# antoineleeman/robust-nonlinear-mpc

Measured on AMD Instinct MI355X. Metric: QP solves/sec (whole node), rockETH N=20 batch=4096 closed-loop RTI MPC step from script x0, higher is better.
Workload: dtype f64

## Files before the change

__graft_entry__.py:

```python
import os
import subprocess
import sys

ROOT = os.path.dirname(os.path.abspath(__file__))
CSRC = os.path.join(ROOT, "robust-nonlinear-mpc_amd", "csrc")
if ROOT not in sys.path:
    sys.path.insert(0, ROOT)


MFMA_FLAGS = ["-mllvm", "-amdgpu-mfma-vgpr-form"]


def _stale(target, sources):
    if not os.path.exists(target):
        return True
    t = os.path.getmtime(target)
    return any(os.path.getmtime(s) > t for s in sources)


def build(force=False):
    so = os.path.join(CSRC, "libslsqp_hip.so")
    srcs = [os.path.join(CSRC, f) for f in os.listdir(CSRC) if f.endswith((".hip", ".hpp"))] + [os.path.join(ROOT, "include", "slsqp.h")]
    if force or _stale(so, srcs):
        cmd = ["hipcc", "-O3", "--offload-arch=gfx950", "-std=c++17", "-shared", "-fPIC", "-Wno-unused-result", "-Wno-unused-value", "-Wno-pass-failed", *MFMA_FLAGS,
               "-o", so, os.path.join(CSRC, "slsqp_api.hip")] + os.environ.get("SLSQP_EXTRA_FLAGS", "").split()
        subprocess.check_call(cmd)
    so2 = os.path.join(CSRC, "libslsqp_hip_dims62.so")
    if force or _stale(so2, srcs):
        subprocess.check_call(["hipcc", "-O3", "--offload-arch=gfx950", "-std=c++17", "-shared", "-fPIC", "-Wno-unused-result", "-Wno-unused-value", "-Wno-pass-failed", *MFMA_FLAGS,
                               "-DSLSQP_EXTRA_DIMS=X(6,2)", "-o", so2, os.path.join(CSRC, "slsqp_api.hip")])
    from oracle import oracle as O
    O.build(force)
    import robust_nonlinear_mpc_amd
    from robust_nonlinear_mpc_amd import _lib
    import ctypes
    lib = ctypes.CDLL(_lib.SO_PATH)
    missing = [e for e in _lib.EXPORTS if not hasattr(lib, e)]
    if missing:
        raise RuntimeError(f"libslsqp_hip.so lacks symbols: {missing}")


def smoke():
    import numpy as np
    sys.path.insert(0, os.path.join(ROOT, "tests"))
    from problems import make_instance, run_oracle_fastsls, run_gpu_fastsls
    insts = [make_instance("pendulum", s, 0.5) for s in range(4)]
    ref = [run_oracle_fastsls(i, rti_steps=1) for i in insts]
    out = run_gpu_fastsls(insts, rti_steps=1)
    for b, r in enumerate(ref):
        assert bool(out["success"][b]) == bool(r["success"])
        if not r["success"]:
            continue
        err = np.max(np.abs(out["primal_vec"][b] - r["primal_vec"])) / max(1.0, np.max(np.abs(r["primal_vec"])))
        assert err < 1e-6, f"instance {b}: primal mismatch {err}"
        assert np.allclose(out["backoff"][b], r["backoff"], rtol=1e-6, atol=1e-9)
    assert out["success"].any()
    print("smoke ok: max KKT stationarity", float(out["kkt"][:, 0].max()))


if __name__ == "__main__":
    build()
    print("build ok")
```

robust-nonlinear-mpc_amd/csrc/slsqp_kernels.hpp:

```cpp
#pragma once
#include <hip/hip_runtime.h>

#include "dynamics.hpp"
#include "wave_la.hpp"

namespace slsqp {

constexpr double BIGB = 1e19;
__device__ __forceinline__ double nan_max(double a, double b) { return fmax(a, b == b ? b : INFINITY); }
constexpr double EPS_PIN = 1e-10;
constexpr int ST_INIT = -1;

#ifndef NE_MFMA
#define NE_MFMA 1
#endif
#ifndef NE_GJ_MFMA
#define NE_GJ_MFMA 1
#endif

struct Costs {
    const double *Qd, *Rd, *Qfd;
    const double *Qregd, *Rregd, *Qregfd;
    double prox;
};

template <int NX, int NU>
struct Lay {
    static constexpr int NZ = NX + NU, NI = 2 * NZ, NIF = 2 * NX, SR = NX + NI;
    __host__ __device__ static int n(int N) { return NZ * N + NX; }
    __host__ __device__ static int mb(int N) { return N * SR + NIF; }
};

struct QpArgs {
    int B, N;
    const double *A, *Bm;
    const double *q;
    const double *ubg, *lbg;
    const double *x0val;
    const int *run;
    Costs cst;
    double *Linv;
    double *ws;
    double *state;
    double *primal;
    double *dual;
    double *cost;
    double *pin_dual;
    double *kkt;
    int *status, *iters;
    int max_iter;
    double eps;
    double init_s, init_lam;
    int warm_rounds;
    int warm;
    const double *prox;
    int prox_stride;
    unsigned long long *inst_launches;
    int *qpstat;
    int stat_slot;
    int snap_take;
    int snap_use;
    double snap_mu;
    double call_id;
    const double *call_ids;
    int as_first;
    int as_rounds;
    int *diag;
    const int *shift_stepno;
    int warm_shift;
    int as_warm_max_set;
    int as_warm_last;
    double pinf_eps;
    int as_max_viol;
    int n_refine;
    double early_ctol;
};

__host__ __device__ inline size_t kkt_doubles(size_t B) { return 8 * B + 2 + 2 * B; }
__host__ __device__ inline double *x0_record(double *kkt, int B) { return kkt + (size_t)8 * B; }

template <int NX, int NU>
struct QpLds {
    static constexpr int NZ = NX + NU, MM = NX * NX;
    static constexpr bool MFMA = (NE_MFMA != 0) && NX >= 13;
    static constexpr int oA = 0, oL1 = MM, oP = MFMA ? MM : 2 * MM, oQ = oP + MM, oB = oQ + MM, oPiS = oB + NX * NU, oVS = oPiS + NZ + NX,
                         oWp = oVS + NZ + NX, oT1 = oWp + NX, oT2 = oT1 + NX, oT3 = oT2 + NX, TOTAL = oT3 + NX + 1;
};
template <int NX, int NU>
__host__ __device__ constexpr int qp_lds_doubles(int) { return QpLds<NX, NU>::TOTAL; }

__host__ __device__ inline size_t qp_ws_doubles(int n, int N, int NX) { return (size_t)20 * n + (size_t)5 * N * NX; }

template <int NX, int NU>
struct NeG {
    const double *A, *Bm, *ub, *lb;
    double *Linv, *PI, *V, *G, *W;
    double *UF;
    int N;
};

// ... 310 lines not shown
        r.lo = -ub[N * SR + NX + i];
    }
    r.fr = e >= NX;
    r.fu = r.fr && r.hi < BIGB;
    r.fl = r.fr && r.lo > -BIGB;
    return r;
}

enum { P_INIT = 0, P_PRED = 1, P_CORR = 2, P_POL0 = 3, P_POL1 = 4, P_POL2 = 5, P_DONE = 6 };
#ifndef STALL_WINDOW
#define STALL_WINDOW 6
#endif
#ifndef STALL_MIN_IT
#define STALL_MIN_IT 24
#endif
#ifndef STALL_FACTOR
#define STALL_FACTOR 0.5
#endif
#ifndef AS_DELTA
#define AS_DELTA 1e-13
#endif
#ifndef RES_ONLY_TOL
#define RES_ONLY_TOL 1e-9
#endif
struct QpState {
    double phase, it, status, mu, smu, qscale, mtot, pol_round, pol_fail, warm, kst, kbox, ksign, pst, pbox, psign, ticks, fticks, tight, pad;
    double snap_call, snap_mu, snap_used, pad2;
    double mode, cold_as, nviol, path;
    unsigned long long seth[4];
    double kmin, fact_call, act1_ok, uf_valid;
    double res_only, tbox, stall_ref, stall_it;
};
static_assert(sizeof(QpState) == 40 * sizeof(double), "QpState size");

#ifndef LAUNDER_B
#define LAUNDER_B(b) asm volatile("" : "+s"(b))
#endif
template <int NX, int NU>
__device__ __forceinline__ NeG<NX, NU> make_neg(const QpArgs &a, int b) {
    using L = Lay<NX, NU>;
    const int N = a.N, n = L::n(N), mb = L::mb(N);
    double *ws = a.ws + (size_t)b * qp_ws_doubles(n, N, NX);
    NeG<NX, NU> g;
    g.A = a.A + (size_t)b * N * NX * NX; g.Bm = a.Bm + (size_t)b * N * NX * NU;
    g.ub = a.ubg + (size_t)b * mb; g.lb = a.lbg + (size_t)b * mb;
    g.Linv = a.Linv + (size_t)b * N * NX * NX; g.PI = ws + 8 * (size_t)n; g.V = ws + 9 * (size_t)n; g.G = ws + 10 * (size_t)n;
    g.W = ws + 12 * (size_t)n; g.UF = ws + 19 * (size_t)n + 4 * (size_t)N * NX; g.N = N;
    return g;
}

struct FwdPlan { bool factor; double eflag, delta; int k0, ks; };
__device__ __forceinline__ FwdPlan fwd_plan(const QpState *st, int phase, int N) {
    FwdPlan p;
    p.factor = (phase == P_INIT || phase == P_PRED || phase == P_POL0);
    p.eflag = (phase == P_INIT || phase >= P_POL0) ? 1.0 : 0.0;
    p.delta = (phase == P_POL0 || (phase == P_INIT && st->mode == 0.0)) ? AS_DELTA : 0.0;
    p.k0 = (phase == P_POL0) ? (int)st->kmin : 0;
    p.ks = (phase == P_POL0 && st->uf_valid != 0.0 && p.k0 < N) ? p.k0 : 0;
    return p;
}

__device__ __noinline__ int x0_gate(double *kkt, int B, int b, int slot, double vmax, int lane) {
    double *xr = x0_record(kkt, B);
    if (lane == 0) xr[2 + (size_t)b * 2 + slot] = vmax;
    return (vmax > fmax(1e-9, xr[0]) || !(vmax < INFINITY)) ? 1 : 0;
}

template <int NX, int NU>
__device__ __forceinline__ void phase_update(const QpArgs &a, int first, int b, int lane, double *sm = nullptr) {
    using L = Lay<NX, NU>;
    constexpr int NZ = L::NZ, SR = L::SR;
    const int N = a.N, n = L::n(N), mb = L::mb(N);
    const double *ub = a.ubg + (size_t)b * mb, *qg = a.q + (size_t)b * n;
    double *ws = a.ws + (size_t)b * qp_ws_doubles(n, N, NX);
    double *Z = ws, *SU = Z + n, *SL = SU + n, *LU = SL + n, *LL = LU + n, *GC = LL + n, *CU = GC + n, *CL = CU + n;
    double *PI = CL + n, *V = PI + n, *G = V + n, *ACT = G + n, *W = ACT + n, *NUA = W + N * NX, *NUP = NUA + N * NX;
    double *SZ = NUP + N * NX, *SSU = SZ + n, *SSL = SSU + n, *SLU = SSL + n, *SLL = SLU + n, *SGC = SLL + n, *SNUA = SGC + n;
    double *ACT1 = SNUA + N * NX;
    double *ACT2 = ws + 19 * (size_t)n + 5 * (size_t)N * NX;
    Costs cst = a.cst;
    cst.prox = a.prox ? a.prox[(size_t)b * a.prox_stride] : 0.0;
    const double call_id = a.call_ids ? a.call_ids[b] : a.call_id;
    QpState *stp = (QpState *)a.state + b;
    auto restore_iterate = [&](double mu_snap) {
        const double smin = fmax(sqrt(fmax(mu_snap, 0.0)), 1e-3);
#pragma unroll 4
        for (int e = lane; e < n; e += 64) {
            const Elem el = elem_of<NX, NU>(e, n, N, ub, qg, cst);
            const double z = (e < NX) ? a.x0val[(size_t)b * NX + e] : SZ[e], su = SSU[e], sl = SSL[e];
            Z[e] = z; GC[e] = SGC[e];
            SU[e] = el.fu ? fmax(el.hi - z, fmin(su, smin)) : 1.0; LU[e] = el.fu ? SLU[e] : 0.0;
            SL[e] = el.fl ? fmax(z - el.lo, fmin(sl, smin)) : 1.0; LL[e] = el.fl ? SLL[e] : 0.0;
        }
        for (int o = lane; o < N * NX; o += 64) NUA[o] = SNUA[o];
    };

    if (first) {
        int status = ST_INIT;
        double viol = -INFINITY;
        if (lane < NX) {
            const double xv = a.x0val[(size_t)b * NX + lane];
            viol = fmax(xv - ub[NX + lane], -ub[NX + NZ + lane] - xv);
            if (isnan(viol)) viol = INFINITY;
        }
        if (x0_gate(a.kkt, a.B, b, a.stat_slot, wla::wave_max(viol), lane)) status = 2;
        int okbits = (int)stp->act1_ok;
        int age1 = (okbits >> 2) & 255, age2 = (okbits >> 10) & 255;
        if (a.stat_slot == 0 && a.snap_use == 0 && a.warm_shift && (!a.shift_stepno || a.shift_stepno[b] > 0)) { age1 = min(age1 + 1, 255); age2 = min(age2 + 1, 255); }
        okbits = (okbits & 3) | (age1 << 2) | (age2 << 10);
        const bool from_act1 = a.warm && status == ST_INIT && a.stat_slot == 0 && a.snap_use == 0 && (okbits & 1);
        bool warm = a.warm && status == ST_INIT && (from_act1 || (((int)stp->status == 0) && ((int)stp->phase == P_DONE)));
        const bool have_act2 = a.warm && status == ST_INIT && a.stat_slot == 1 && a.as_warm_last > 0 && (okbits & 2);
        bool from_act2 = have_act2 && (a.as_warm_last >= 2 || !warm);
        bool big_set = false;
        if (warm && !from_act1 && !from_act2 && a.snap_use != 0 && a.as_warm_max_set > 0) {
            double cnt = 0.0;
            for (int e = lane; e < n; e += 64) cnt += (ACT[e] != 0.0) ? 1.0 : 0.0;
            big_set = wla::wave_sum(cnt) > (double)a.as_warm_max_set;
            if (big_set) { if (have_act2) { from_act2 = true; big_set = false; } else warm = false; }
        }
        if (from_act2) warm = true;
        const double *prev = a.primal + (size_t)b * n;
        const bool keep_fact = warm && !from_act1 && !from_act2 && a.snap_use != 0 && stp->fact_call == call_id && call_id != 0.0;
        double set_changed = 0.0;
        double qscale = 0.0, mtot = 0.0;
#pragma unroll 4
        for (int e = lane; e < n; e += 64) {
            const Elem el = elem_of<NX, NU>(e, n, N, ub, qg, cst);
            qscale = fmax(qscale, fabs(el.q));
            mtot += (el.fu ? 1.0 : 0.0) + (el.fl ? 1.0 : 0.0);
            if (warm) {
                const double ac_old = ACT[e];
                const double *src = from_act1 ? ACT1 : ACT2;
                int es = e + (from_act1 ? age1 : age2) * NZ;
                while (es >= n) es -= NZ;
                double ac = (from_act1 || from_act2) ? src[es] : ac_old;
                if ((ac > 0.0 && !el.fu) || (ac < 0.0 && !el.fl) || !el.fr) ac = 0.0;
                if (ac != ac_old) set_changed = 1.0;
                const double zp = (e < NX) ? a.x0val[(size_t)b * NX + e] : prev[e];
                const double z0 = ac > 0.0 ? el.hi : (ac < 0.0 ? el.lo : zp);
                const double pi = (el.fr && ac == 0.0) ? wla::fast_rcp(el.pd) : 0.0;
                ACT[e] = ac; PI[e] = pi; V[e] = (pi != 0.0) ? -pi * el.q : z0;
            } else {
                const double z0 = (e < NX) ? a.x0val[(size_t)b * NX + e] : 0.0;
                const double pi = el.fr ? wla::fast_rcp(el.pd) : 0.0;
                PI[e] = pi; V[e] = (pi != 0.0) ? -pi * el.q : z0; Z[e] = z0;
            }
        }
        qscale = fmax(1.0, wla::wave_max(qscale));
        mtot = fmax(1.0, wla::wave_sum(mtot));
        const bool skip_fact = keep_fact && wla::wave_max(set_changed) == 0.0;
        if (lane == 0) {
            QpState s0;
            s0.phase = (status == ST_INIT) ? (warm ? P_POL0 : P_INIT) : P_DONE; s0.it = 0; s0.status = status; s0.mu = 0; s0.smu = 0; s0.qscale = qscale;
            s0.mtot = mtot; s0.pol_round = 0; s0.pol_fail = 0; s0.warm = warm ? 1.0 : 0.0; s0.kst = 0; s0.kbox = 0; s0.ksign = 0; s0.pst = -1; s0.pbox = -1; s0.psign = -1; s0.ticks = 0; s0.fticks = 0; s0.tight = 0; s0.pad = 0;
            s0.snap_call = stp->snap_call; s0.snap_mu = stp->snap_mu; s0.snap_used = 0; s0.pad2 = 0;
            s0.mode = (a.as_first && !big_set) ? 0.0 : 1.0; s0.cold_as = big_set ? 1.0 : 0.0; s0.nviol = 0; s0.path = warm ? (from_act2 ? 20.0 : 10.0) : (big_set ? 1.0 : 0.0);
            s0.seth[0] = s0.seth[1] = s0.seth[2] = s0.seth[3] = 0ULL; s0.kmin = skip_fact ? (double)N : 0.0; s0.fact_call = 0; s0.act1_ok = (double)okbits; s0.uf_valid = 0; s0.res_only = 0; s0.tbox = 0; s0.stall_ref = 0; s0.stall_it = 0;
            *stp = s0;
            a.status[b] = status; a.iters[b] = 0;
#ifdef QP_DIAG_SPAN
            if (a.diag) for (int i = 0; i < 32; i++) a.diag[((size_t)b * 2 + a.stat_slot) * 32 + i] = -1;
#endif
            if (status != ST_INIT && a.qpstat) {
                int *qs = a.qpstat + ((size_t)b * 2 + a.stat_slot) * 8;
                for (int i = 0; i < 8; i++) qs[i] = 0;
                qs[6] = status;
            }
        }
        return;
    }

    QpState s = *stp;
    int phase = (int)s.phase;
    if (phase == P_DONE) return;
    int status = (int)s.status, it = (int)s.it;
    const double qscale = s.qscale, mtot = s.mtot, ptol = 1e-9 * qscale;
    double tol = (s.tight != 0.0 ? fmin(a.eps, 1e-9) : a.eps) * qscale;
    bool polished = false, start_iter = false, fall_back = false;

    bool as_from_init = false;
    if (phase == P_INIT && s.mode == 0.0) {
#pragma unroll 4
        for (int e = lane; e < n; e += 64) {
            const Elem el = elem_of<NX, NU>(e, n, N, ub, qg, cst);
            const double gc = G[e];
            CU[e] = el.fr ? -(el.q + gc) * wla::fast_rcp(el.pd) : Z[e];
            CL[e] = gc; ACT[e] = 0.0;
        }
        for (int o = lane; o < N * NX; o += 64) NUP[o] = W[o];
        s.cold_as = 1.0; s.warm = 2.0; s.pol_round = 0.0; s.pol_fail = 0.0; s.nviol = 0.0;
        as_from_init = true;
        phase = P_POL0;
        wla::wsync_mem();
    }
    if (phase == P_INIT) {
        for (int o = lane; o < N * NX; o += 64) NUA[o] = W[o];
#pragma unroll 4
        for (int e = lane; e < n; e += 64) {
            const Elem el = elem_of<NX, NU>(e, n, N, ub, qg, cst);
            const double gc = G[e];
            const double z = el.fr ? -(el.q + gc) * wla::fast_rcp(el.pd) : Z[e];
            GC[e] = gc; Z[e] = z;
            const double lam0 = a.init_lam > 0.0 ? a.init_lam : fmax(1.0, 0.1 * qscale);
            SU[e] = el.fu ? fmax(el.hi - z, a.init_s) : 1.0; LU[e] = el.fu ? lam0 : 0.0;
            SL[e] = el.fl ? fmax(z - el.lo, a.init_s) : 1.0; LL[e] = el.fl ? lam0 : 0.0;
        }
        start_iter = true;
    } else if (phase == P_PRED) {
        double amin = 1.0, S0 = 0.0, S1 = 0.0, S2 = 0.0;
#pragma unroll 4
        for (int e = lane; e < n; e += 64) {
            const Elem el = elem_of<NX, NU>(e, n, N, ub, qg, cst);
            const double dz = V[e] - PI[e] * G[e];
            const double z = Z[e], su = SU[e], sl = SL[e], lu = LU[e], ll = LL[e];
            double cu = 0.0, cl = 0.0;
            if (el.fu) {
                const double ru = z + su - el.hi, dsu = -ru - dz, dlu = -lu + (lu * ru + lu * dz) * wla::fast_rcp(su);
                if (dsu < 0) amin = fmin(amin, -su * wla::fast_rcp(dsu));
                if (dlu < 0) amin = fmin(amin, -lu * wla::fast_rcp(dlu));
                S0 += su * lu; S1 += su * dlu + lu * dsu; cu = dsu * dlu; S2 += cu;
            }
            if (el.fl) {
                const double rl = el.lo - z + sl, dsl = -rl + dz, dll = -ll + (ll * rl - ll * dz) * wla::fast_rcp(sl);
                if (dsl < 0) amin = fmin(amin, -sl * wla::fast_rcp(dsl));
                if (dll < 0) amin = fmin(amin, -ll * wla::fast_rcp(dll));
                S0 += sl * ll; S1 += sl * dll + ll * dsl; cl = dsl * dll; S2 += cl;
            }
            CU[e] = cu; CL[e] = cl;
        }
        const double aaff = wla::wave_min(amin);
        S0 = wla::wave_sum(S0); S1 = wla::wave_sum(S1); S2 = wla::wave_sum(S2);
        const double muaff = (S0 + aaff * (S1 + aaff * S2)) / mtot;
        double sig = muaff / s.mu; sig = sig * sig * sig;
        const double smu = sig * s.mu;
        s.smu = smu;
#pragma unroll 4
        for (int e = lane; e < n; e += 64) {
            const Elem el = elem_of<NX, NU>(e, n, N, ub, qg, cst);
            const double z = Z[e], su = SU[e], sl = SL[e], lu = LU[e], ll = LL[e];
            double rr = el.fr ? el.pd * z + el.q + GC[e] + lu - ll : 0.0;
            if (el.fu) rr += (-(su * lu + CU[e] - smu) + lu * (z + su - el.hi)) * wla::fast_rcp(su);
            if (el.fl) rr -= (-(sl * ll + CL[e] - smu) + ll * (el.lo - z + sl)) * wla::fast_rcp(sl);
            V[e] = -PI[e] * rr;
        }
        phase = P_CORR;
    } else if (phase == P_CORR) {
        const double smu = s.smu;
        double amin = 1e300;
#pragma unroll 4
        for (int e = lane; e < n; e += 64) {
            const Elem el = elem_of<NX, NU>(e, n, N, ub, qg, cst);
            const double dz = V[e] - PI[e] * G[e];
            const double z = Z[e], su = SU[e], sl = SL[e], lu = LU[e], ll = LL[e];
            if (el.fu) {
                const double ru = z + su - el.hi, dsu = -ru - dz;
                const double dlu = (-(su * lu + CU[e] - smu) + lu * ru + lu * dz) * wla::fast_rcp(su);
                if (dsu < 0) amin = fmin(amin, -su * wla::fast_rcp(dsu));
                if (dlu < 0) amin = fmin(amin, -lu * wla::fast_rcp(dlu));
            }
            if (el.fl) {
                const double rl = el.lo - z + sl, dsl = -rl + dz;
                const double dll = (-(sl * ll + CL[e] - smu) + ll * rl - ll * dz) * wla::fast_rcp(sl);
                if (dsl < 0) amin = fmin(amin, -sl * wla::fast_rcp(dsl));
                if (dll < 0) amin = fmin(amin, -ll * wla::fast_rcp(dll));
            }
        }
        const double alpha = fmin(1.0, 0.99 * wla::wave_min(amin));
#pragma unroll 4
        for (int e = lane; e < n; e += 64) {
            const Elem el = elem_of<NX, NU>(e, n, N, ub, qg, cst);
            const double gg = G[e];
            const double dz = V[e] - PI[e] * gg;
            const double z = Z[e], su = SU[e], sl = SL[e], lu = LU[e], ll = LL[e];
            if (el.fu) {
                const double ru = z + su - el.hi, dsu = -ru - dz;
                const double dlu = (-(su * lu + CU[e] - smu) + lu * ru + lu * dz) * wla::fast_rcp(su);
                SU[e] = su + alpha * dsu; LU[e] = lu + alpha * dlu;
            }
            if (el.fl) {
                const double rl = el.lo - z + sl, dsl = -rl + dz;
                const double dll = (-(sl * ll + CL[e] - smu) + ll * rl - ll * dz) * wla::fast_rcp(sl);
                SL[e] = sl + alpha * dsl; LL[e] = ll + alpha * dll;
            }
            Z[e] = z + alpha * dz; GC[e] += alpha * gg;
        }
        for (int o = lane; o < N * NX; o += 64) NUA[o] += alpha * W[o];
        it++;
        start_iter = true;
    } else if (phase == P_POL2 && s.res_only != 0.0 && stp->pbox < RES_ONLY_TOL * qscale) {
        polished = true; status = 0; s.kst = s.pst; s.kbox = s.tbox; s.ksign = s.psign; s.pbox = stp->pbox; s.res_only = 0.0;
        phase = P_DONE;
    } else {
        s.res_only = 0.0;
        const bool firstp = (phase == P_POL0);
        const double max_rounds = (s.warm == 1.0) ? (double)a.warm_rounds : (s.warm == 2.0 ? (double)a.as_rounds : 8.0);
        const bool look = (phase == P_POL0 && s.pol_fail == 0.0 && s.pol_round < max_rounds);
        const bool fused_look = look && sm != nullptr;
        if (!as_from_init && !fused_look) {
#pragma unroll 4
            for (int e = lane; e < n; e += 64) {
                const double gg = G[e];
                CU[e] = V[e] - PI[e] * gg;
                CL[e] = (firstp ? 0.0 : CL[e]) + gg;
            }
            for (int o = lane; o < N * NX; o += 64) NUP[o] = (firstp ? 0.0 : NUP[o]) + W[o];
            wla::wsync_mem();
        }
        auto viol_at = [&](int e, double tolv) -> double {
            if (e < NX || e >= n || ACT[e] != 0.0) return 0.0;
            const Elem el = elem_of<NX, NU>(e, n, N, ub, qg, cst);
            const double zn = CU[e];
            double v = 0.0;
            if (el.fu) v = fmax(v, zn - el.hi);
            if (el.fl) v = fmax(v, el.lo - zn);
            return v > tolv ? v : 0.0;
        };
        auto plan_set = [&](double tolv, double &nv, unsigned long long &hash) -> double {
            int in_viol = 0;
            for (int o = lane; o < N * NU; o += 64) {
                const int e = (o / NU) * NZ + NX + (o % NU);
                in_viol |= (viol_at(e, tolv) > 0.0) ? 1 : 0;
            }
            const bool any_in = wla::wave_or(in_viol) != 0;
            double changed = 0.0, viols = 0.0, kfirst = 1e9;
            unsigned long long hv = 0ULL;
#pragma unroll 2
            for (int e = lane; e < n; e += 64) {
                const Elem el = elem_of<NX, NU>(e, n, N, ub, qg, cst);
                const double zn = CU[e], gr = el.pd * zn + el.q + CL[e], ac = ACT[e];
                double nac = ac;
                if (ac > 0.0 && gr > tolv) nac = 0.0;
                if (ac < 0.0 && -gr > tolv) nac = 0.0;
                if (ac == 0.0 && el.fr) {
                    const double vu = el.fu ? zn - el.hi : 0.0, vl = el.fl ? el.lo - zn : 0.0, v = fmax(vu, vl);
                    if (v > tolv) {
                        viols += 1.0;
                        bool take = true;
                        if ((e % NZ) < NX) take = !any_in && (v >= viol_at(e - NZ, tolv)) && (v >= viol_at(e + NZ, tolv));
                        if (take) nac = vu > vl ? 1.0 : -1.0;
                    }
                }
                if (nac != ac) { changed += 1.0; kfirst = fmin(kfirst, (double)max(0, e / NZ - ((e % NZ) < NX ? 1 : 0))); }
                if (nac != 0.0) {
                    unsigned long long x = (unsigned long long)(2 * e + (nac > 0.0 ? 1 : 0)) + 0x9E3779B97F4A7C15ULL;
                    x = (x ^ (x >> 30)) * 0xBF58476D1CE4E5B9ULL; x = (x ^ (x >> 27)) * 0x94D049BB133111EBULL; hv ^= x ^ (x >> 31);
                }
                G[e] = nac;
            }
#pragma unroll
            for (int o = 32; o > 0; o >>= 1) {
                const unsigned lo32 = __shfl_xor((unsigned)(hv & 0xFFFFFFFFULL), o), hi32 = __shfl_xor((unsigned)(hv >> 32), o);
                hv ^= ((unsigned long long)hi32 << 32) | lo32;
            }
            hash = hv | 1ULL;
            nv = wla::wave_sum(viols);
            s.kmin = fmin(wla::wave_min(kfirst), (double)N);
            return wla::wave_sum(changed);
        };
        auto seen_before = [&](unsigned long long hsh) -> bool {
            const bool rep = (hsh == s.seth[0]) || (hsh == s.seth[1]) || (hsh == s.seth[2]) || (hsh == s.seth[3]);
            s.seth[3] = s.seth[2]; s.seth[2] = s.seth[1]; s.seth[1] = s.seth[0]; s.seth[0] = hsh;
            return rep;
        };
        auto apply_set = [&]() {
            wla::wsync_mem();
#pragma unroll 4
            for (int e = lane; e < n; e += 64) {
                const Elem el = elem_of<NX, NU>(e, n, N, ub, qg, cst);
                const double zn = CU[e], ac = G[e];
                const double z0 = ac > 0.0 ? el.hi : (ac < 0.0 ? el.lo : zn);
                const double pi = (el.fr && ac == 0.0) ? wla::fast_rcp(el.pd) : 0.0;
                ACT[e] = ac; PI[e] = pi; V[e] = (pi != 0.0) ? -pi * el.q : z0;
            }
        };
        bool again = false, give_up = false;
        double tvst = 0.0, tvbox = 0.0, tvsign = 0.0;
        auto fused_plan = [&](double tolv, double &nv, unsigned long long &hash) -> double {
            double *sV = sm, *sN = sm + n;
            int in_viol = 0;
            double viols = 0.0;
#pragma unroll 2
            for (int e = lane; e < n; e += 64) {
                const Elem el = elem_of<NX, NU>(e, n, N, ub, qg, cst);
                double zn, cl;
                if (as_from_init) { zn = CU[e]; cl = CL[e]; }
                else {
                    const double gg = G[e];
                    zn = V[e] - PI[e] * gg; cl = (firstp ? 0.0 : CL[e]) + gg;
                    CU[e] = zn; CL[e] = cl;
                }
                const double gr = el.pd * zn + el.q + cl, ac = ACT[e];
                if (el.fr && ac == 0.0) tvst = nan_max(tvst, fabs(gr));
                if (el.fu) tvbox = nan_max(tvbox, zn - el.hi);
                if (el.fl) tvbox = nan_max(tvbox, el.lo - zn);
                if (ac > 0.0) tvsign = nan_max(tvsign, gr);
                if (ac < 0.0) tvsign = nan_max(tvsign, -gr);
                double nac = ac;
                if (ac > 0.0 && gr > tolv) nac = 0.5;
                if (ac < 0.0 && -gr > tolv) nac = 0.5;
                double v = 0.0;
                if (ac == 0.0 && el.fr) {
                    const double vu = el.fu ? zn - el.hi : 0.0, vl = el.fl ? el.lo - zn : 0.0, vm = fmax(vu, vl);
                    if (vm > tolv) { v = vu > vl ? vm : -vm; viols += 1.0; if ((e % NZ) >= NX) in_viol = 1; }
                }
                sV[e] = v; sN[e] = nac;
            }
            if (!as_from_init) for (int o = lane; o < N * NX; o += 64) NUP[o] = (firstp ? 0.0 : NUP[o]) + W[o];
            wla::wsync();
            const bool any_in = wla::wave_or(in_viol) != 0;
            double changed = 0.0, kfirst = 1e9;
#ifdef QP_DIAG_SPAN
            double klast = -1.0;
#endif
            unsigned long long hv = 0ULL;
#pragma unroll 2
            for (int e = lane; e < n; e += 64) {
                const double v = sV[e];
                double nac = sN[e];
                bool chg = (nac == 0.5);
                if (chg) nac = 0.0;
                if (v != 0.0) {
                    bool take = true;
                    if ((e % NZ) < NX) {
                        const double va = fabs(v), vp = (e - NZ >= NX) ? fabs(sV[e - NZ]) : 0.0, vn = (e + NZ < n) ? fabs(sV[e + NZ]) : 0.0;
                        take = !any_in && va >= vp && va >= vn;
                    }
                    if (take) { nac = v > 0.0 ? 1.0 : -1.0; chg = true; }
                }
                if (chg) { changed += 1.0; kfirst = fmin(kfirst, (double)max(0, e / NZ - ((e % NZ) < NX ? 1 : 0))); }
#ifdef QP_DIAG_SPAN
                if (chg) klast = fmax(klast, (double)min(N - 1, e / NZ));
#endif
                if (nac != 0.0) {
                    unsigned long long x = (unsigned long long)(2 * e + (nac > 0.0 ? 1 : 0)) + 0x9E3779B97F4A7C15ULL;
                    x = (x ^ (x >> 30)) * 0xBF58476D1CE4E5B9ULL; x = (x ^ (x >> 27)) * 0x94D049BB133111EBULL; hv ^= x ^ (x >> 31);
                }
                sN[e] = nac;
            }
#pragma unroll
            for (int o = 32; o > 0; o >>= 1) {
                const unsigned lo32 = __shfl_xor((unsigned)(hv & 0xFFFFFFFFULL), o), hi32 = __shfl_xor((unsigned)(hv >> 32), o);
                hv ^= ((unsigned long long)hi32 << 32) | lo32;
            }
            hash = hv | 1ULL;
            nv = wla::wave_sum(viols);
            s.kmin = fmin(wla::wave_min(kfirst), (double)N);
#ifdef QP_DIAG_SPAN
            {
                const double kl = wla::wave_max(klast);
                const int r = (int)s.pol_round;
                if (lane == 0 && a.diag && r < 16 && kl >= 0.0) { int *dg = a.diag + (((size_t)b * 2 + a.stat_slot) * 16 + r) * 2; dg[0] = (int)s.kmin; dg[1] = (int)kl; }
            }
#endif
            return wla::wave_sum(changed);
        };
        auto fused_apply = [&]() {
            const double *sN = sm + n;
#pragma unroll 4
            for (int e = lane; e < n; e += 64) {
                const Elem el = elem_of<NX, NU>(e, n, N, ub, qg, cst);
                const double ac = sN[e];
                const double z0 = ac > 0.0 ? el.hi : (ac < 0.0 ? el.lo : 0.0);
                const double pi = (el.fr && ac == 0.0) ? wla::fast_rcp(el.pd) : 0.0;
                ACT[e] = ac; PI[e] = pi; V[e] = (pi != 0.0) ? -pi * el.q : ((e < NX) ? a.x0val[(size_t)b * NX + e] : z0);
            }
        };
        if (look) {
            double nv = 0.0;
            unsigned long long hsh = 0ULL;
            const double changed = fused_look ? fused_plan(a.early_ctol * qscale, nv, hsh) : plan_set(a.early_ctol * qscale, nv, hsh);
            again = changed > 0.0;
            if (again && s.warm > 0.0 && seen_before(hsh)) { again = false; give_up = true; }
            if (s.warm > 0.0 && (nv > (double)a.as_max_viol || (s.pol_round > 0.0 && nv > 2.0 * s.nviol + 8.0 && nv > 24.0))) { again = false; give_up = true; }
            s.nviol = nv;
            if (again) { s.pol_round += 1.0; if (fused_look) fused_apply(); else apply_set(); s.uf_valid = 1.0; }
            if (fused_look) wla::wsync_mem();
        } else if (phase == P_POL0 && s.warm > 0.0) give_up = true;
        if (again) {
            phase = P_POL0;
        } else if (give_up) {
            fall_back = true;
        } else if (phase != P_POL2) {
    #pragma unroll 4
        for (int e = lane; e < n; e += 64) {
                const Elem el = elem_of<NX, NU>(e, n, N, ub, qg, cst);
                const double pi = PI[e], zn = CU[e];
                const double r1 = (pi != 0.0) ? el.pd * zn + el.q + CL[e] : 0.0;
                V[e] = zn - pi * r1;
            }
            s.res_only = 0.0;
            if (fused_look && a.n_refine <= 1 && s.pol_fail == 0.0) {
                const double wst = wla::wave_max(tvst), wbox = wla::wave_max(tvbox), wsign = wla::wave_max(tvsign);
                if (wst < ptol && wbox < ptol && wsign < ptol) { s.res_only = 1.0; s.pst = wst; s.tbox = wbox; s.psign = wsign; }
            }
            if (phase == P_POL0) { s.pad = 0.0; phase = (a.n_refine <= 1) ? P_POL2 : P_POL1; }
            else { s.pad += 1.0; phase = (s.pad + 1.0 >= (double)a.n_refine) ? P_POL2 : P_POL1; }
        } else {
            double vst = 0.0, vbox = 0.0, vsign = 0.0;
    #pragma unroll 4
        for (int e = lane; e < n; e += 64) {
                const Elem el = elem_of<NX, NU>(e, n, N, ub, qg, cst);
                const double zn = CU[e], gr = el.pd * zn + el.q + CL[e], ac = ACT[e];
                if (el.fr && ac == 0.0) vst = nan_max(vst, fabs(gr));
                if (el.fu) vbox = nan_max(vbox, zn - el.hi);
                if (el.fl) vbox = nan_max(vbox, el.lo - zn);
                if (ac > 0.0) vsign = nan_max(vsign, gr);
                if (ac < 0.0) vsign = nan_max(vsign, -gr);
            }
            vst = wla::wave_max(vst); vbox = wla::wave_max(vbox); vsign = wla::wave_max(vsign);
            s.pst = vst; s.psign = vsign;
            const bool pf = s.pol_fail != 0.0;
            const double eqres = stp->pbox;
            s.pbox = eqres;
            if (!pf && vst < ptol && vbox < ptol && vsign < ptol && eqres < 1e-6 * qscale) {
                polished = true; status = 0; s.kst = vst; s.kbox = vbox; s.ksign = vsign;
                phase = P_DONE;
            } else if (!pf && vst < ptol && s.pol_round < max_rounds) {
                double nv = 0.0;
                unsigned long long hsh = 0ULL;
                plan_set(ptol, nv, hsh);
                if (s.warm > 0.0 && seen_before(hsh)) fall_back = true;
                else { s.pol_round += 1.0; s.nviol = nv; apply_set(); phase = P_POL0; s.uf_valid = 0.0; }
            } else if (s.warm > 0.0) {
                fall_back = true;
            } else if (s.tight == 0.0 && a.eps > 1e-9 && status == 4) {
                s.tight = 1.0; s.pol_round = 0.0; s.pol_fail = 0.0; tol = fmin(a.eps, 1e-9) * qscale;
                start_iter = true;
            } else phase = P_DONE;
        }
    }

    if (fall_back) {
        const bool try_cold_as = a.as_first == 1 && s.cold_as == 0.0 && s.warm == 1.0;
        s.pol_round = 0.0; s.pol_fail = 0.0; s.seth[0] = s.seth[1] = s.seth[2] = s.seth[3] = 0ULL; s.uf_valid = 0.0;
        if (!try_cold_as && a.snap_use && s.snap_call == call_id && call_id != 0.0) {
            s.warm = -1.0; s.path = 10.0 * floor(s.path / 10.0) + 2.0;
            restore_iterate(s.snap_mu);
            s.snap_used = 1.0;
            start_iter = true;
        } else {
            const double w10 = 10.0 * floor(s.path / 10.0);
            if (try_cold_as) { s.mode = 0.0; s.path = w10 + 3.0; s.warm = -1.0; }
            else { s.mode = 1.0; s.path = w10 + 1.0; s.warm = -1.0; }
    #pragma unroll 4
            for (int e = lane; e < n; e += 64) {
                const Elem el = elem_of<NX, NU>(e, n, N, ub, qg, cst);
                const double z0 = (e < NX) ? a.x0val[(size_t)b * NX + e] : 0.0;
                const double pi = el.fr ? wla::fast_rcp(el.pd) : 0.0;
                PI[e] = pi; V[e] = (pi != 0.0) ? -pi * el.q : z0; Z[e] = z0;
            }
            phase = P_INIT;
        }
    }

    if (start_iter) {
        wla::wsync_mem();
        double rmax = 0.0, musum = 0.0;
#pragma unroll 4
        for (int e = lane; e < n; e += 64) {
            const Elem el = elem_of<NX, NU>(e, n, N, ub, qg, cst);
            const double z = Z[e], su = SU[e], sl = SL[e], lu = LU[e], ll = LL[e];
            const double rd = el.fr ? el.pd * z + el.q + GC[e] + lu - ll : 0.0;
            const double ru = el.fu ? z + su - el.hi : 0.0, rl = el.fl ? el.lo - z + sl : 0.0;
            rmax = fmax(rmax, fmax(fabs(rd), fmax(fabs(ru), fabs(rl))));
            musum += (el.fu ? su * lu : 0.0) + (el.fl ? sl * ll : 0.0);
            const double Wu = el.fu ? lu * wla::fast_rcp(su) : 0.0, Wl = el.fl ? ll * wla::fast_rcp(sl) : 0.0;
            const double pi = el.fr ? wla::fast_rcp(el.pd + Wu + Wl) : 0.0;
            const double tu = el.fu ? -lu + Wu * ru : 0.0, tl = el.fl ? -ll + Wl * rl : 0.0;
            PI[e] = pi; V[e] = -pi * (rd + tu - tl);
        }
        const double res = wla::wave_max(rmax);
        const double mu = wla::wave_sum(musum) / mtot;
        s.mu = mu; s.kst = res;
        bool farkas = false;
        if (a.pinf_eps > 0.0 && it >= 4 && res == res) {
            double ymax = 0.0, aty = 0.0, sup = 0.0;
#pragma unroll 4
            for (int e = lane; e < n; e += 64) {
                const Elem el = elem_of<NX, NU>(e, n, N, ub, qg, cst);
                const double lu = el.fu ? LU[e] : 0.0, ll = el.fl ? LL[e] : 0.0, gc = GC[e];
                ymax = fmax(ymax, fmax(lu, ll));
                if (el.fr) { aty = fmax(aty, fabs(gc + lu - ll)); sup += (el.fu ? el.hi * lu : 0.0) - (el.fl ? el.lo * ll : 0.0); }
                else sup -= a.x0val[(size_t)b * NX + e] * gc;
            }
            const double *lbv = a.lbg + (size_t)b * mb;
            for (int o = lane; o < N * NX; o += 64) {
                const double nu = NUA[o];
                const int r = (o / NX) * SR + (o % NX);
                ymax = fmax(ymax, fabs(nu));
                sup += 0.5 * (ub[r] + lbv[r]) * nu;
            }
            ymax = wla::wave_max(ymax); aty = wla::wave_max(aty); sup = wla::wave_sum(sup);
            farkas = ymax > 0.0 && aty <= a.pinf_eps * ymax && sup < -a.pinf_eps * ymax;
        }
        if (a.snap_take && s.pad2 == 0.0 && mu <= a.snap_mu * qscale && mu >= 1e-2 * a.snap_mu * qscale && res == res) {
#pragma unroll 4
            for (int e = lane; e < n; e += 64) { SZ[e] = Z[e]; SSU[e] = SU[e]; SSL[e] = SL[e]; SLU[e] = LU[e]; SLL[e] = LL[e]; SGC[e] = GC[e]; }
            for (int o = lane; o < N * NX; o += 64) SNUA[o] = NUA[o];
            s.pad2 = 1.0; s.snap_call = call_id; s.snap_mu = mu;
        }
        bool stalled = false;
        {
            const double phi = fmax(res, mu);
            if (s.stall_ref == 0.0) { s.stall_ref = phi; s.stall_it = (double)it; }
            else if ((double)it - s.stall_it >= (double)STALL_WINDOW) {
                stalled = it >= STALL_MIN_IT && phi > STALL_FACTOR * s.stall_ref;
                s.stall_ref = phi; s.stall_it = (double)it;
            }
        }
        if (farkas) { status = 5; phase = P_DONE; }
        else if (!(res == res) || !(mu == mu) || res > 1e30) { status = 3; phase = P_DONE; }
        else if (res < tol && mu < tol) {
            status = 4;
    #pragma unroll 4
        for (int e = lane; e < n; e += 64) {
                const Elem el = elem_of<NX, NU>(e, n, N, ub, qg, cst);
                const double z = Z[e], lam = LU[e] - LL[e];
                const bool aU = el.fu && (lam > el.hi - z);
                const bool aL = el.fl && !aU && (-lam > z - el.lo);
                const double z0 = aU ? el.hi : (aL ? el.lo : z);
                const double pi = (el.fr && !aU && !aL) ? wla::fast_rcp(el.pd) : 0.0;
                ACT[e] = aU ? 1.0 : (aL ? -1.0 : 0.0); PI[e] = pi; V[e] = (pi != 0.0) ? -pi * el.q : z0;
            }
            phase = P_POL0; s.kmin = 0.0; s.uf_valid = 0.0;
        } else if (it >= a.max_iter || stalled) {
            status = (s.tight != 0.0 && status == 4) ? 4 : 1; phase = P_DONE;
        }
        else phase = P_PRED;
    }

    if (phase == P_DONE) {
        wla::wsync_mem();
        double *pr = a.primal + (size_t)b * n, *du = a.dual + (size_t)b * mb;
        double csum = 0.0, nact = 0.0;
        const bool ok = (status == 0 || status == 4);
        if (ok) {
    #pragma unroll 4
        for (int e = lane; e < n; e += 64) {
                const Elem el = elem_of<NX, NU>(e, n, N, ub, qg, cst);
                double zv, yu, yl, gv;
                if (polished) {
                    zv = CU[e]; gv = CL[e];
                    const double gr = el.pd * zv + el.q + gv, ac = ACT[e];
                    yu = ac > 0.0 ? fmax(-gr, 0.0) : 0.0;
                    yl = ac < 0.0 ? fmax(gr, 0.0) : 0.0;
                } else { zv = Z[e]; gv = GC[e]; yu = el.fu ? LU[e] : 0.0; yl = el.fl ? LL[e] : 0.0; }
                pr[e] = zv;
                nact += (yu > 0.0 ? 1.0 : 0.0) + (yl > 0.0 ? 1.0 : 0.0);
                csum += 0.5 * el.pd * zv * zv + el.q * zv;
                const int k = e / NZ, i = e % NZ;
                if (k < N) { du[k * SR + NX + i] = yu; du[k * SR + NX + NZ + i] = yl; }
                else { du[N * SR + i] = yu; du[N * SR + NX + i] = yl; }
                if (e < NX && a.pin_dual) a.pin_dual[(size_t)b * NX + e] = -(el.pd * zv + el.q + gv);
            }
            const double *nus = polished ? NUP : NUA;
            for (int o = lane; o < N * NX; o += 64) du[(o / NX) * SR + (o % NX)] = nus[o];
            if (polished && a.stat_slot == 0 && a.snap_use == 0) {
                for (int e = lane; e < n; e += 64) ACT1[e] = ACT[e];
                s.act1_ok = (double)((((int)s.act1_ok | 1)) & ~(255 << 2));
            }
            if (polished && a.stat_slot == 1) {
                for (int e = lane; e < n; e += 64) ACT2[e] = ACT[e];
                s.act1_ok = (double)((((int)s.act1_ok | 2)) & ~(255 << 10));
            }
        }
        if (polished) s.fact_call = call_id;
        csum = wla::wave_sum(csum);
        nact = wla::wave_sum(nact);
        if (lane == 0) {
            if (a.qpstat) {
                int *qs = a.qpstat + ((size_t)b * 2 + a.stat_slot) * 8;
                qs[0] = it; qs[1] = (int)stp->ticks; qs[2] = (int)stp->fticks; qs[3] = (int)nact; qs[4] = (int)s.path / 10;
                qs[5] = (int)s.pol_round; qs[6] = status; qs[7] = (int)s.path % 10;
            }
            if (ok) a.cost[b] = csum;
            a.status[b] = status;
            a.iters[b] = it;
            double *kk = a.kkt + (size_t)b * 8;
            kk[0] = s.kst; kk[1] = s.kbox; kk[2] = s.ksign; kk[3] = s.mu; kk[4] = s.pst; kk[5] = s.pbox; kk[6] = stp->fticks; kk[7] = stp->ticks;
        }
    }
    if (lane == 0) { s.phase = phase; s.it = it; s.status = status; s.ticks = stp->ticks; s.fticks = stp->fticks; *stp = s; }
}

#ifndef QP_PERSIST_WAVES_PER_SIMD
#define QP_PERSIST_WAVES_PER_SIMD 3
#endif

template <int NX, int NU, bool MX = false>
__device__ __forceinline__ int qp_solve_dev(const QpArgs &a, int b, int lane, double *sm, int max_ticks, int resume = 0, unsigned long long deadline = ~0ULL,
                                            const unsigned *fin_count = nullptr, unsigned cut_count = 0xFFFFFFFFu) {
    if (!resume) {
        if (a.run && !a.run[b]) {
            if (a.qpstat && lane < 8) a.qpstat[((size_t)b * 2 + a.stat_slot) * 8 + lane] = (lane == 6) ? -1 : 0;
            return 1;
        }
// ... 1229 lines not shown
```

Measured before the change: 1.538 million.

## Fuse IPM iterate update with residual and Farkas passes in QP phase update

The interior-point iterate update (init, predictor step, snapshot restore) now computes residuals, complementarity sums, the PI/V factors and the Farkas infeasibility statistics in the same per-element loop, so the separate re-read passes are skipped. The polishing correction also folds the V refinement into the plan loop and reuses the fused plan/apply for refinement rounds. The aim is fewer global memory sweeps over the workspace per IPM iteration. In exchange it adds register pressure, extra wave syncs before snapshot and polish loops, and subtle ordering changes such as the Farkas test now using the post-increment iteration count. An unfused build is kept behind a macro.

```diff
diff --git a/__graft_entry__.py b/__graft_entry__.py
--- a/__graft_entry__.py
+++ b/__graft_entry__.py
@@ -29,6 +29,10 @@
     if force or _stale(so2, srcs):
         subprocess.check_call(["hipcc", "-O3", "--offload-arch=gfx950", "-std=c++17", "-shared", "-fPIC", "-Wno-unused-result", "-Wno-unused-value", "-Wno-pass-failed", *MFMA_FLAGS,
                                "-DSLSQP_EXTRA_DIMS=X(6,2)", "-o", so2, os.path.join(CSRC, "slsqp_api.hip")])
+    so3 = os.path.join(CSRC, "libslsqp_hip_unfused.so")
+    if force or _stale(so3, srcs):
+        subprocess.check_call(["hipcc", "-O3", "--offload-arch=gfx950", "-std=c++17", "-shared", "-fPIC", "-Wno-unused-result", "-Wno-unused-value", "-Wno-pass-failed", *MFMA_FLAGS,
+                               "-DQP_FUSED_PASSES=0", "-o", so3, os.path.join(CSRC, "slsqp_api.hip")])
     from oracle import oracle as O
     O.build(force)
     import robust_nonlinear_mpc_amd
diff --git a/robust-nonlinear-mpc_amd/csrc/slsqp_kernels.hpp b/robust-nonlinear-mpc_amd/csrc/slsqp_kernels.hpp
--- a/robust-nonlinear-mpc_amd/csrc/slsqp_kernels.hpp
+++ b/robust-nonlinear-mpc_amd/csrc/slsqp_kernels.hpp
@@ -16,6 +16,9 @@
 #endif
 #ifndef NE_GJ_MFMA
 #define NE_GJ_MFMA 1
+#endif
+#ifndef QP_FUSED_PASSES
+#define QP_FUSED_PASSES 1
 #endif
 
 struct Costs {
@@ -492,6 +495,7 @@
     cst.prox = a.prox ? a.prox[(size_t)b * a.prox_stride] : 0.0;
     const double call_id = a.call_ids ? a.call_ids[b] : a.call_id;
     QpState *stp = (QpState *)a.state + b;
+#if !QP_FUSED_PASSES
     auto restore_iterate = [&](double mu_snap) {
         const double smin = fmax(sqrt(fmax(mu_snap, 0.0)), 1e-3);
 #pragma unroll 4
@@ -504,6 +508,7 @@
         }
         for (int o = lane; o < N * NX; o += 64) NUA[o] = SNUA[o];
     };
+#endif
 
     if (first) {
         int status = ST_INIT;
@@ -589,6 +594,50 @@
     double tol = (s.tight != 0.0 ? fmin(a.eps, 1e-9) : a.eps) * qscale;
     bool polished = false, start_iter = false, fall_back = false;
 
+#if QP_FUSED_PASSES
+    double it_rmax = 0.0, it_musum = 0.0, fk_ymax = 0.0, fk_aty = 0.0, fk_sup = 0.0;
+    bool iter_ready = false, fk_on = false;
+    auto iter_begin = [&]() __attribute__((always_inline)) { iter_ready = true; fk_on = a.pinf_eps > 0.0 && it >= 4; asm volatile("" : "+v"(lane)); };
+    auto iter_elem = [&](int e, const Elem &el, double z, double su, double sl, double lu, double ll, double gc) __attribute__((always_inline)) {
+        const double rd = el.fr ? el.pd * z + el.q + gc + lu - ll : 0.0;
+        const double ru = el.fu ? z + su - el.hi : 0.0, rl = el.fl ? el.lo - z + sl : 0.0;
+        it_rmax = fmax(it_rmax, fmax(fabs(rd), fmax(fabs(ru), fabs(rl))));
+        it_musum += (el.fu ? su * lu : 0.0) + (el.fl ? sl * ll : 0.0);
+        const double Wu = el.fu ? lu * wla::fast_rcp(su) : 0.0, Wl = el.fl ? ll * wla::fast_rcp(sl) : 0.0;
+        const double pi = el.fr ? wla::fast_rcp(el.pd + Wu + Wl) : 0.0;
+        const double tu = el.fu ? -lu + Wu * ru : 0.0, tl = el.fl ? -ll + Wl * rl : 0.0;
+        PI[e] = pi; V[e] = -pi * (rd + tu - tl);
+        if (fk_on) {
+            const double flu = el.fu ? lu : 0.0, fll = el.fl ? ll : 0.0;
+            fk_ymax = fmax(fk_ymax, fmax(flu, fll));
+            if (el.fr) { fk_aty = fmax(fk_aty, fabs(gc + flu - fll)); fk_sup += (el.fu ? el.hi * flu : 0.0) - (el.fl ? el.lo * fll : 0.0); }
+            else fk_sup -= a.x0val[(size_t)b * NX + e] * gc;
+        }
+    };
+    auto iter_nu = [&](int o, double nu) __attribute__((always_inline)) {
+        if (fk_on) {
+            const double *lbv = a.lbg + (size_t)b * mb;
+            const int r = (o / NX) * SR + (o % NX);
+            fk_ymax = fmax(fk_ymax, fabs(nu));
+            fk_sup += 0.5 * (ub[r] + lbv[r]) * nu;
+        }
+    };
+    auto restore_iterate = [&](double mu_snap) __attribute__((always_inline)) {
+        const double smin = fmax(sqrt(fmax(mu_snap, 0.0)), 1e-3);
+        iter_begin();
+#pragma unroll 1
+        for (int e = lane; e < n; e += 64) {
+            const Elem el = elem_of<NX, NU>(e, n, N, ub, qg, cst);
+            const double z = (e < NX) ? a.x0val[(size_t)b * NX + e] : SZ[e], su = SSU[e], sl = SSL[e], gc = SGC[e];
+            const double sun = el.fu ? fmax(el.hi - z, fmin(su, smin)) : 1.0, lun = el.fu ? SLU[e] : 0.0;
+            const double sln = el.fl ? fmax(z - el.lo, fmin(sl, smin)) : 1.0, lln = el.fl ? SLL[e] : 0.0;
+            Z[e] = z; GC[e] = gc; SU[e] = sun; LU[e] = lun; SL[e] = sln; LL[e] = lln;
+            iter_elem(e, el, z, sun, sln, lun, lln, gc);
+        }
+        for (int o = lane; o < N * NX; o += 64) { const double nu = SNUA[o]; NUA[o] = nu; iter_nu(o, nu); }
+    };
+#endif
+
     bool as_from_init = false;
     if (phase == P_INIT && s.mode == 0.0) {
 #pragma unroll 4
@@ -605,6 +654,21 @@
         wla::wsync_mem();
     }
     if (phase == P_INIT) {
+#if QP_FUSED_PASSES
+        iter_begin();
+        const double lam0 = a.init_lam > 0.0 ? a.init_lam : fmax(1.0, 0.1 * qscale);
+#pragma unroll 1
+        for (int e = lane; e < n; e += 64) {
+            const Elem el = elem_of<NX, NU>(e, n, N, ub, qg, cst);
+            const double gc = G[e];
+            const double z = el.fr ? -(el.q + gc) * wla::fast_rcp(el.pd) : Z[e];
+            const double su = el.fu ? fmax(el.hi - z, a.init_s) : 1.0, lu = el.fu ? lam0 : 0.0;
+            const double sl = el.fl ? fmax(z - el.lo, a.init_s) : 1.0, ll = el.fl ? lam0 : 0.0;
+            GC[e] = gc; Z[e] = z; SU[e] = su; LU[e] = lu; SL[e] = sl; LL[e] = ll;
+            iter_elem(e, el, z, su, sl, lu, ll, gc);
+        }
+        for (int o = lane; o < N * NX; o += 64) { const double nu = W[o]; NUA[o] = nu; iter_nu(o, nu); }
+#else
         for (int o = lane; o < N * NX; o += 64) NUA[o] = W[o];
 #pragma unroll 4
         for (int e = lane; e < n; e += 64) {
@@ -616,6 +680,7 @@
             SU[e] = el.fu ? fmax(el.hi - z, a.init_s) : 1.0; LU[e] = el.fu ? lam0 : 0.0;
             SL[e] = el.fl ? fmax(z - el.lo, a.init_s) : 1.0; LL[e] = el.fl ? lam0 : 0.0;
         }
+#endif
         start_iter = true;
     } else if (phase == P_PRED) {
         double amin = 1.0, S0 = 0.0, S1 = 0.0, S2 = 0.0;
@@ -677,6 +742,34 @@
             }
         }
         const double alpha = fmin(1.0, 0.99 * wla::wave_min(amin));
+#if QP_FUSED_PASSES
+        it++;
+        iter_begin();
+#pragma unroll 2
+        for (int e = lane; e < n; e += 64) {
+            const Elem el = elem_of<NX, NU>(e, n, N, ub, qg, cst);
+            const double gg = G[e];
+            const double dz = V[e] - PI[e] * gg;
+            const double z = Z[e];
+            double su = SU[e], sl = SL[e], lu = LU[e], ll = LL[e];
+            if (el.fu) {
+                const double ru = z + su - el.hi, dsu = -ru - dz;
+                const double dlu = (-(su * lu + CU[e] - smu) + lu * ru + lu * dz) * wla::fast_rcp(su);
+                su = su + alpha * dsu; lu = lu + alpha * dlu;
+                SU[e] = su; LU[e] = lu;
+            }
+            if (el.fl) {
+                const double rl = el.lo - z + sl, dsl = -rl + dz;
+                const double dll = (-(sl * ll + CL[e] - smu) + ll * rl - ll * dz) * wla::fast_rcp(sl);
+                sl = sl + alpha * dsl; ll = ll + alpha * dll;
+                SL[e] = sl; LL[e] = ll;
+            }
+            const double zn = z + alpha * dz, gc = GC[e] + alpha * gg;
+            Z[e] = zn; GC[e] = gc;
+            iter_elem(e, el, zn, su, sl, lu, ll, gc);
+        }
+        for (int o = lane; o < N * NX; o += 64) { const double nu = NUA[o] + alpha * W[o]; NUA[o] = nu; iter_nu(o, nu); }
+#else
 #pragma unroll 4
         for (int e = lane; e < n; e += 64) {
             const Elem el = elem_of<NX, NU>(e, n, N, ub, qg, cst);
@@ -697,6 +790,7 @@
         }
         for (int o = lane; o < N * NX; o += 64) NUA[o] += alpha * W[o];
         it++;
+#endif
         start_iter = true;
     } else if (phase == P_POL2 && s.res_only != 0.0 && stp->pbox < RES_ONLY_TOL * qscale) {
         polished = true; status = 0; s.kst = s.pst; s.kbox = s.tbox; s.ksign = s.psign; s.pbox = stp->pbox; s.res_only = 0.0;
@@ -786,21 +880,36 @@
         };
         bool again = false, give_up = false;
         double tvst = 0.0, tvbox = 0.0, tvsign = 0.0;
-        auto fused_plan = [&](double tolv, double &nv, unsigned long long &hash) -> double {
+        auto fused_plan = [&](double tolv, double &nv, unsigned long long &hash, bool corr = false) -> double {
             double *sV = sm, *sN = sm + n;
             int in_viol = 0;
             double viols = 0.0;
+            const bool have_zn = as_from_init || corr;
 #pragma unroll 2
             for (int e = lane; e < n; e += 64) {
                 const Elem el = elem_of<NX, NU>(e, n, N, ub, qg, cst);
                 double zn, cl;
-                if (as_from_init) { zn = CU[e]; cl = CL[e]; }
+#if QP_FUSED_PASSES
+                double pi;
+                if (have_zn) { zn = CU[e]; cl = CL[e]; pi = PI[e]; }
+                else {
+                    const double gg = G[e];
+                    pi = PI[e];
+                    zn = V[e] - pi * gg; cl = (firstp ? 0.0 : CL[e]) + gg;
+                    CU[e] = zn; CL[e] = cl;
+                }
+#else
+                if (have_zn) { zn = CU[e]; cl = CL[e]; }
                 else {
                     const double gg = G[e];
                     zn = V[e] - PI[e] * gg; cl = (firstp ? 0.0 : CL[e]) + gg;
                     CU[e] = zn; CL[e] = cl;
                 }
+#endif
                 const double gr = el.pd * zn + el.q + cl, ac = ACT[e];
+#if QP_FUSED_PASSES
+                V[e] = zn - pi * ((pi != 0.0) ? gr : 0.0);
+#endif
                 if (el.fr && ac == 0.0) tvst = nan_max(tvst, fabs(gr));
                 if (el.fu) tvbox = nan_max(tvbox, zn - el.hi);
                 if (el.fl) tvbox = nan_max(tvbox, el.lo - zn);
@@ -860,12 +969,12 @@
             {
                 const double kl = wla::wave_max(klast);
                 const int r = (int)s.pol_round;
-                if (lane == 0 && a.diag && r < 16 && kl >= 0.0) { int *dg = a.diag + (((size_t)b * 2 + a.stat_slot) * 16 + r) * 2; dg[0] = (int)s.kmin; dg[1] = (int)kl; }
+                if (lane == 0 && a.diag && r < 16 && kl >= 0.0 && !corr) { int *dg = a.diag + (((size_t)b * 2 + a.stat_slot) * 16 + r) * 2; dg[0] = (int)s.kmin; dg[1] = (int)kl; }
             }
 #endif
             return wla::wave_sum(changed);
         };
-        auto fused_apply = [&]() {
+        auto fused_apply = [&](bool corr = false) {
             const double *sN = sm + n;
 #pragma unroll 4
             for (int e = lane; e < n; e += 64) {
@@ -873,7 +982,7 @@
                 const double ac = sN[e];
                 const double z0 = ac > 0.0 ? el.hi : (ac < 0.0 ? el.lo : 0.0);
                 const double pi = (el.fr && ac == 0.0) ? wla::fast_rcp(el.pd) : 0.0;
-                ACT[e] = ac; PI[e] = pi; V[e] = (pi != 0.0) ? -pi * el.q : ((e < NX) ? a.x0val[(size_t)b * NX + e] : z0);
+                ACT[e] = ac; PI[e] = pi; V[e] = (pi != 0.0) ? -pi * el.q : ((e < NX) ? (corr ? CU[e] : a.x0val[(size_t)b * NX + e]) : z0);
             }
         };
         if (look) {
@@ -892,12 +1001,14 @@
         } else if (give_up) {
             fall_back = true;
         } else if (phase != P_POL2) {
+            if (!(QP_FUSED_PASSES && fused_look)) {
     #pragma unroll 4
         for (int e = lane; e < n; e += 64) {
                 const Elem el = elem_of<NX, NU>(e, n, N, ub, qg, cst);
                 const double pi = PI[e], zn = CU[e];
                 const double r1 = (pi != 0.0) ? el.pd * zn + el.q + CL[e] : 0.0;
                 V[e] = zn - pi * r1;
+            }
             }
             s.res_only = 0.0;
             if (fused_look && a.n_refine <= 1 && s.pol_fail == 0.0) {
@@ -929,9 +1040,16 @@
             } else if (!pf && vst < ptol && s.pol_round < max_rounds) {
                 double nv = 0.0;
                 unsigned long long hsh = 0ULL;
+#if QP_FUSED_PASSES
+                const bool fused_corr = sm != nullptr;
+                if (fused_corr) fused_plan(ptol, nv, hsh, true); else plan_set(ptol, nv, hsh);
+                if (s.warm > 0.0 && seen_before(hsh)) fall_back = true;
+                else { s.pol_round += 1.0; s.nviol = nv; if (fused_corr) fused_apply(true); else apply_set(); phase = P_POL0; s.uf_valid = 0.0; }
+#else
                 plan_set(ptol, nv, hsh);
                 if (s.warm > 0.0 && seen_before(hsh)) fall_back = true;
                 else { s.pol_round += 1.0; s.nviol = nv; apply_set(); phase = P_POL0; s.uf_valid = 0.0; }
+#endif
             } else if (s.warm > 0.0) {
                 fall_back = true;
             } else if (s.tight == 0.0 && a.eps > 1e-9 && status == 4) {
@@ -965,6 +1083,20 @@
     }
 
     if (start_iter) {
+#if QP_FUSED_PASSES
+        if (!iter_ready) {
+            wla::wsync_mem();
+            iter_begin();
+#pragma unroll 1
+            for (int e = lane; e < n; e += 64) {
+                const Elem el = elem_of<NX, NU>(e, n, N, ub, qg, cst);
+                const double z = Z[e], su = SU[e], sl = SL[e], lu = LU[e], ll = LL[e], gc = GC[e];
+                iter_elem(e, el, z, su, sl, lu, ll, gc);
+            }
+            for (int o = lane; o < N * NX; o += 64) iter_nu(o, NUA[o]);
+        }
+        const double rmax = it_rmax, musum = it_musum;
+#else
         wla::wsync_mem();
         double rmax = 0.0, musum = 0.0;
 #pragma unroll 4
@@ -980,10 +1112,17 @@
             const double tu = el.fu ? -lu + Wu * ru : 0.0, tl = el.fl ? -ll + Wl * rl : 0.0;
             PI[e] = pi; V[e] = -pi * (rd + tu - tl);
         }
+#endif
         const double res = wla::wave_max(rmax);
         const double mu = wla::wave_sum(musum) / mtot;
         s.mu = mu; s.kst = res;
         bool farkas = false;
+#if QP_FUSED_PASSES
+        if (fk_on) {
+            const double ymax = wla::wave_max(fk_ymax), aty = wla::wave_max(fk_aty), sup = wla::wave_sum(fk_sup);
+            farkas = res == res && ymax > 0.0 && aty <= a.pinf_eps * ymax && sup < -a.pinf_eps * ymax;
+        }
+#else
         if (a.pinf_eps > 0.0 && it >= 4 && res == res) {
             double ymax = 0.0, aty = 0.0, sup = 0.0;
 #pragma unroll 4
@@ -1004,7 +1143,11 @@
             ymax = wla::wave_max(ymax); aty = wla::wave_max(aty); sup = wla::wave_sum(sup);
             farkas = ymax > 0.0 && aty <= a.pinf_eps * ymax && sup < -a.pinf_eps * ymax;
         }
+#endif
         if (a.snap_take && s.pad2 == 0.0 && mu <= a.snap_mu * qscale && mu >= 1e-2 * a.snap_mu * qscale && res == res) {
+#if QP_FUSED_PASSES
+            wla::wsync_mem();
+#endif
 #pragma unroll 4
             for (int e = lane; e < n; e += 64) { SZ[e] = Z[e]; SSU[e] = SU[e]; SSL[e] = SL[e]; SLU[e] = LU[e]; SLL[e] = LL[e]; SGC[e] = GC[e]; }
             for (int o = lane; o < N * NX; o += 64) SNUA[o] = NUA[o];
@@ -1023,6 +1166,9 @@
         else if (!(res == res) || !(mu == mu) || res > 1e30) { status = 3; phase = P_DONE; }
         else if (res < tol && mu < tol) {
             status = 4;
+#if QP_FUSED_PASSES
+            wla::wsync_mem();
+#endif
     #pragma unroll 4
         for (int e = lane; e < n; e += 64) {
                 const Elem el = elem_of<NX, NU>(e, n, N, ub, qg, cst);
```

Result: slower. 1.496 million (-2.8%).
